# ucb-bar/Accelerated-TinyMPC

Measured on AMD Instinct MI355X. Metric: MPC solves/sec (batched quadrotor nx=12,nu=4,N=30), higher is better.
Workload: dtype f32; 1 GPU; quadrotor_tracking batched 65536 instances per GPU, cold-start tiny_solve, early_exit (tol 1e-3, max_iter 100); nx=12, nu=4, N=30, instances_per_gpu=65536, instances_total=65536, parallelism=batch-shard x1, world_size_seen=1, backend=none (single process), kernel=tile16<12,4,30,exact>, max_iters=85

## Files before the change

accelerated-tinympc_amd/csrc/admm_tile16.hip:

```cpp
#include "rowlane_math.h"
#include <cstdlib>

namespace tinympc
{

typedef float f32x16 __attribute__((ext_vector_type(16)));
#ifndef TINY_T16_ABLATE
#define TINY_T16_ABLATE 0
#endif
#ifndef TINY_T16_CQ
#define TINY_T16_CQ 1
#endif
#ifndef TINY_T16_BADDR
#define TINY_T16_BADDR 1
#endif
#ifndef TINY_T16_PADTAB
#define TINY_T16_PADTAB 1
#endif
#ifndef TINY_T16_XPOSE
#define TINY_T16_XPOSE 1
#endif
#ifndef TINY_T16_SCHED
#define TINY_T16_SCHED 1
#endif
#ifndef TINY_T16_LINES
#define TINY_T16_LINES 1
#endif
#ifndef TINY_T16_STAMP
#define TINY_T16_STAMP 0
#endif

#if TINY_T16_ABLATE == 1
__device__ __forceinline__ f32x4 t16_fake4(float a, float b, f32x4 c) { c[0] += a; c[1] += b; c[2] += a; c[3] += b; return c; }
#define TINY_MFMA4(a, b, c) t16_fake4((a), (b), (c))
#define TINY_MFMA1(a, b, c) __builtin_amdgcn_mfma_f32_16x16x1f32((a), (b), (c), 0, 0, 0)
#else
#define TINY_MFMA4(a, b, c) __builtin_amdgcn_mfma_f32_16x16x4f32((a), (b), (c), 0, 0, 0)
#define TINY_MFMA1(a, b, c) __builtin_amdgcn_mfma_f32_16x16x1f32((a), (b), (c), 0, 0, 0)
#endif

template <int V>
__device__ __forceinline__ void gather12(float (&t)[12], const f32x16 &p0, const f32x16 &p1, const f32x16 &p2)
{
#pragma unroll
    for (int b = 0; b < 4; b++)
    {
        t[b] = p0[4 * b + V];
        t[4 + b] = p1[4 * b + V];
        t[8 + b] = p2[4 * b + V];
    }
}
template <int V>
__device__ __forceinline__ void gather4(float (&t)[4], const f32x16 &p)
{
#pragma unroll
    for (int b = 0; b < 4; b++) t[b] = p[4 * b + V];
}

typedef float f32x2 __attribute__((ext_vector_type(2)));
template <int B>
__device__ __forceinline__ f32x4 blk(const f32x16 &p) { return __builtin_shufflevector(p, p, 4 * B, 4 * B + 1, 4 * B + 2, 4 * B + 3); }
__device__ __forceinline__ void gather12v(f32x4 (&t)[12], const f32x16 &p0, const f32x16 &p1, const f32x16 &p2)
{
    t[0] = blk<0>(p0); t[1] = blk<1>(p0); t[2] = blk<2>(p0); t[3] = blk<3>(p0);
    t[4] = blk<0>(p1); t[5] = blk<1>(p1); t[6] = blk<2>(p1); t[7] = blk<3>(p1);
    t[8] = blk<0>(p2); t[9] = blk<1>(p2); t[10] = blk<2>(p2); t[11] = blk<3>(p2);
}
__device__ __forceinline__ void gather4v(f32x4 (&t)[4], const f32x16 &p)
{
    t[0] = blk<0>(p); t[1] = blk<1>(p); t[2] = blk<2>(p); t[3] = blk<3>(p);
}
template <int LO, int CNT, int NN>
__device__ __forceinline__ f32x4 tree_sum4(const f32x4 (&t)[NN])
{
    if constexpr (CNT == 1) return t[LO];
    else
    {
        constexpr int H = CNT / 2;
        return tree_sum4<LO, H>(t) + tree_sum4<LO + H, CNT - H>(t);
    }
}
template <int PLO, int PCNT, int L, int NN>
__device__ __forceinline__ f32x4 ptree_sum4(const f32x4 (&t)[NN])
{
    if constexpr (PCNT == 1) return t[4 * PLO + L];
    else
    {
        constexpr int H = PCNT / 2;
        return ptree_sum4<PLO, H, L>(t) + ptree_sum4<PLO + H, PCNT - H, L>(t);
    }
}
template <int PLAN, int NN>
__device__ __forceinline__ f32x4 reduce4(const f32x4 (&t)[NN])
{
    if constexpr (NN == 1) return t[0];
    else if constexpr (PLAN == PLAN_SEQ)
    {
        f32x4 acc = t[0];
#pragma unroll
        for (int k = 1; k < NN; k++) acc = acc + t[k];
        return acc;
    }
    else if constexpr (PLAN == PLAN_TREE) return tree_sum4<0, NN>(t);
    else
    {
        static_assert(NN % 4 == 0, "packed VEC plan: whole packets only");
        constexpr int NPK = NN / 4;
        const f32x4 s0 = ptree_sum4<0, NPK, 0>(t), s1 = ptree_sum4<0, NPK, 1>(t), s2 = ptree_sum4<0, NPK, 2>(t), s3 = ptree_sum4<0, NPK, 3>(t);
        return (s0 + s2) + (s1 + s3);
    }
}

template <bool EXACT>
struct TileMath
{
    static constexpr int NX = 12, NU = 4;
    using PL = RowPlans<NX, NU>;
    float A1[3], A2, A3[3], A45, AP[3];
    f32x16 negz;

    __device__ __forceinline__ void load(const float *mats, int g, int c)
    {
        const float *m = mats + 4 * (c & 3) + (c >> 2);
#pragma unroll
        for (int ch = 0; ch < 3; ch++)
        {
            A1[ch] = m[(4 * ch + g) * 16];
            A3[ch] = m[(NX + NU + 4 * ch + g) * 16];
            AP[ch] = m[(2 * NX + 2 * NU + 1 + 4 * ch + g) * 16];
        }
        A2 = m[(NX + g) * 16];
        A45 = m[(2 * NX + NU + g) * 16];
#pragma unroll
        for (int e = 0; e < 16; e++) negz[e] = -0.f;
    }

    struct InFlight
    {
        f32x16 p0, p1, p2, pk;
        f32x4 acc;
    };

    __device__ __forceinline__ void lqr_issue(const float (&s)[3], InFlight &F) const
    {
        if constexpr (EXACT)
        {
            F.p0 = TINY_MFMA1(A1[0], s[0], negz); F.p1 = TINY_MFMA1(A1[1], s[1], negz); F.p2 = TINY_MFMA1(A1[2], s[2], negz);
        }
        else
        {
            f32x4 acc = {-0.f, -0.f, -0.f, -0.f};
            acc = TINY_MFMA4(A1[0], s[0], acc);
            acc = TINY_MFMA4(A1[1], s[1], acc);
            F.acc = TINY_MFMA4(A1[2], s[2], acc);
        }
    }
    __device__ __forceinline__ void lqr_finish(const InFlight &F, float di, float &un, float (&xn)[3]) const
    {
        if constexpr (EXACT)
        {
            static_assert(PL::FWD_XA == PL::FWD_U, "x rows and the u row of a lane are summed in one order (both SEQ for nx = 12, nu = 4)");
            f32x4 t[12];
            gather12v(t, F.p0, F.p1, F.p2);
            const f32x4 acc = reduce4<PL::FWD_XA>(t);
            un = -acc[3] - di;
            const f32x16 pb = TINY_MFMA1(A2, un, negz);
            f32x4 t2[4];
            gather4v(t2, pb);
            const f32x4 xn4 = acc + reduce4<PL::FWD_XB>(t2);
            xn[0] = xn4[0]; xn[1] = xn4[1]; xn[2] = xn4[2];
        }
        else
        {
            un = F.acc[3] - di;
            const f32x4 acc = TINY_MFMA4(A2, un, F.acc);
            xn[0] = acc[0]; xn[1] = acc[1]; xn[2] = acc[2];
        }
    }
    __device__ __forceinline__ void lqr(const float (&s)[3], float di, float &un, float (&xn)[3]) const
    {
        InFlight F;
        lqr_issue(s, F);
        lqr_finish(F, di, un, xn);
    }

    __device__ __forceinline__ void riccati_issue(const float (&p)[3], const f32x4 &lin, InFlight &F) const
    {
        if constexpr (EXACT)
        {
            F.p0 = TINY_MFMA1(A3[0], p[0], negz); F.p1 = TINY_MFMA1(A3[1], p[1], negz); F.p2 = TINY_MFMA1(A3[2], p[2], negz);
            F.pk = TINY_MFMA1(A45, lin[3], negz);
        }
        else
        {
            f32x4 acc = lin;
            acc = TINY_MFMA4(A3[0], p[0], acc);
            acc = TINY_MFMA4(A3[1], p[1], acc);
            F.acc = TINY_MFMA4(A3[2], p[2], acc);
        }
    }
    __device__ __forceinline__ void riccati_finish(const InFlight &F, const f32x4 &lin, float (&pn)[3], float &dd) const
    {
        if constexpr (EXACT)
        {
            f32x4 t4[12];
            gather12v(t4, F.p0, F.p1, F.p2);
            const f32x4 wv = lin + reduce4<PL::BWD_PA>(t4);
            float t[12];
            gather12<3>(t, F.p0, F.p1, F.p2);
            const float wv3 = lin[3] + reduce<PL::BWD_TMP>(t);
            const f32x16 pq = TINY_MFMA1(A45, wv3, negz);
            f32x4 tk4[4];
            gather4v(tk4, F.pk);
            const f32x4 pn4 = wv - reduce4<PL::BWD_PK>(tk4);
            pn[0] = pn4[0]; pn[1] = pn4[1]; pn[2] = pn4[2];
            float tk[4];
            gather4<3>(tk, pq); dd = reduce<PL::BWD_D>(tk);
        }
        else
        {
            const f32x4 nz = {-0.f, -0.f, -0.f, -0.f};
            const f32x4 dq = TINY_MFMA4(A45, F.acc[3], nz);
            const f32x4 acc = TINY_MFMA4(A45, lin[3], F.acc);
            pn[0] = acc[0]; pn[1] = acc[1]; pn[2] = acc[2];
            dd = dq[3];
        }
    }
    __device__ __forceinline__ void riccati(const float (&p)[3], const f32x4 &lin, float (&pn)[3], float &dd) const
    {
        InFlight F;
        riccati_issue(p, lin, F);
        riccati_finish(F, lin, pn, dd);
    }

    __device__ __forceinline__ void terminal(const float (&xr)[3], float (&pt)[3]) const
    {
        if constexpr (EXACT)
        {
            const f32x16 p0 = TINY_MFMA1(AP[0], xr[0], negz), p1 = TINY_MFMA1(AP[1], xr[1], negz), p2 = TINY_MFMA1(AP[2], xr[2], negz);
            float t[12];
            gather12<0>(t, p0, p1, p2); pt[0] = -reduce<PL::TERM>(t);
            gather12<1>(t, p0, p1, p2); pt[1] = -reduce<PL::TERM>(t);
            gather12<2>(t, p0, p1, p2); pt[2] = -reduce<PL::TERM>(t);
        }
        else
        {
            f32x4 acc = {-0.f, -0.f, -0.f, -0.f};
            acc = TINY_MFMA4(AP[0], xr[0], acc);
            acc = TINY_MFMA4(AP[1], xr[1], acc);
            acc = TINY_MFMA4(AP[2], xr[2], acc);
            pt[0] = -acc[0]; pt[1] = -acc[1]; pt[2] = -acc[2];
        }
    }
};

__device__ __forceinline__ float tile_inst_max(float v)
{
    v = fmaxf(v, __shfl_xor(v, 16));
    v = fmaxf(v, __shfl_xor(v, 32));
    return v;
}

__device__ __forceinline__ void acc_put(float &dst, float val) { asm volatile("v_accvgpr_write_b32 %0, %1" : "+a"(dst) : "v"(val)); }
__device__ __forceinline__ float acc_get(const float &src)
{
    float r;
    asm volatile("v_accvgpr_read_b32 %0, %1" : "=v"(r) : "a"(src));
    return r;
}
__device__ __forceinline__ void acc_init(float &dst, float val) { asm volatile("v_accvgpr_write_b32 %0, %1" : "=a"(dst) : "v"(val)); }

typedef __attribute__((address_space(3))) float4 lds_float4;
__device__ __forceinline__ void masked_forward_update(unsigned long long m, float (&a)[4], const f32x4 &tp, float (&bo)[4], const f32x4 &old,
                                                      unsigned sn_addr, const f32x4 &t)
{
    unsigned long long sx;
    asm volatile("s_and_saveexec_b64 %[sx], %[m]\n\t"
                 "v_sub_f32 %[a0], %[p0], %[t0]\n\tv_sub_f32 %[a1], %[p1], %[t1]\n\tv_sub_f32 %[a2], %[p2], %[t2]\n\tv_sub_f32 %[a3], %[p3], %[t3]\n\t"
                 "v_accvgpr_write_b32 %[b0], %[o0]\n\tv_accvgpr_write_b32 %[b1], %[o1]\n\tv_accvgpr_write_b32 %[b2], %[o2]\n\tv_accvgpr_write_b32 %[b3], %[o3]\n\t"
                 "ds_write_b128 %[ad], %[tv]\n\t"
                 "s_mov_b64 exec, %[sx]"
                 : [sx] "=&s"(sx), [a0] "+v"(a[0]), [a1] "+v"(a[1]), [a2] "+v"(a[2]), [a3] "+v"(a[3]), [b0] "+a"(bo[0]), [b1] "+a"(bo[1]),
                   [b2] "+a"(bo[2]), [b3] "+a"(bo[3])
                 : [m] "s"(m), [p0] "v"(tp[0]), [p1] "v"(tp[1]), [p2] "v"(tp[2]), [p3] "v"(tp[3]), [t0] "v"(t[0]), [t1] "v"(t[1]), [t2] "v"(t[2]),
                   [t3] "v"(t[3]), [o0] "v"(old[0]), [o1] "v"(old[1]), [o2] "v"(old[2]), [o3] "v"(old[3]), [ad] "v"(sn_addr), [tv] "v"(t)
                 : "memory", "scc");
}
__device__ __forceinline__ void masked_backward_update(unsigned long long m, float (&pl)[3], float &dr, const float (&pn)[3], float dd)
{
    unsigned long long sx;
    asm volatile("s_and_saveexec_b64 %[sx], %[m]\n\t"
                 "v_accvgpr_write_b32 %[p0], %[n0]\n\tv_accvgpr_write_b32 %[p1], %[n1]\n\tv_accvgpr_write_b32 %[p2], %[n2]\n\tv_mov_b32 %[d], %[dd]\n\t"
                 "s_mov_b64 exec, %[sx]"
                 : [sx] "=&s"(sx), [p0] "+a"(pl[0]), [p1] "+a"(pl[1]), [p2] "+a"(pl[2]), [d] "+v"(dr)
                 : [m] "s"(m), [n0] "v"(pn[0]), [n1] "v"(pn[1]), [n2] "v"(pn[2]), [dd] "v"(dd)
                 : "scc");
}

__device__ __forceinline__ void masked_restore_slack(unsigned long long m, const float (&bo)[4], unsigned sn_addr)
{
    const f32x4 tv = {acc_get(bo[0]), acc_get(bo[1]), acc_get(bo[2]), acc_get(bo[3])};
    unsigned long long sx;
    asm volatile("s_and_saveexec_b64 %[sx], %[m]\n\t"
                 "ds_write_b128 %[ad], %[tv]\n\t"
                 "s_mov_b64 exec, %[sx]"
                 : [sx] "=&s"(sx)
                 : [m] "s"(m), [ad] "v"(sn_addr), [tv] "v"(tv)
                 : "memory", "scc");
}

template <bool EXACT>
__device__ __forceinline__ f32x4 lin_cost4(const f32x4 &cq, const f32x4 &rho4, const f32x4 &t1)
{
    if constexpr (EXACT) return cq - rho4 * t1;
    else return __builtin_elementwise_fma(-rho4, t1, cq);
}

__device__ __forceinline__ f32x4 t16_transpose4(const f32x4 &r)
{
    typedef unsigned u32x2 __attribute__((ext_vector_type(2)));
    const u32x2 a = __builtin_amdgcn_permlane32_swap(__float_as_uint(r[0]), __float_as_uint(r[2]), false, false);
    const u32x2 b = __builtin_amdgcn_permlane32_swap(__float_as_uint(r[1]), __float_as_uint(r[3]), false, false);
    const u32x2 lo = __builtin_amdgcn_permlane16_swap(a[0], b[0], false, false);
    const u32x2 hi = __builtin_amdgcn_permlane16_swap(a[1], b[1], false, false);
    return f32x4{__uint_as_float(lo[0]), __uint_as_float(lo[1]), __uint_as_float(hi[0]), __uint_as_float(hi[1])};
}

constexpr int TILE16_WAVES = 4;
constexpr int TILE16_MAX_TABLE_ROWS = 512;

__device__ __forceinline__ void t16_pair_lines(const f32x4 &e, const f32x4 &o, f32x4 &lo8, f32x4 &hi8)
{
#pragma unroll
    for (int k = 0; k < 4; k++)
    {
        lo8[k] = __int_as_float(__builtin_amdgcn_update_dpp(__float_as_int(e[k]), __float_as_int(o[k]), 0x128, 0xf, 0xc, false));
        hi8[k] = __int_as_float(__builtin_amdgcn_update_dpp(__float_as_int(o[k]), __float_as_int(e[k]), 0x128, 0xf, 0x3, false));
    }
}

#if TINY_T16_STAMP && !defined(TINY_T16_PI_UNIT)
constexpr int T16_STAMP_TILES = 32;
__device__ unsigned long long *t16_stamp_buf;
__device__ int t16_stamp_slots;
__device__ __forceinline__ void t16_stamp(int wslot, int k, int field, unsigned long long v)
{
    unsigned long long *const buf = t16_stamp_buf;
    if (buf && wslot < t16_stamp_slots && k < T16_STAMP_TILES && (threadIdx.x & 63) == 0) buf[((size_t)wslot * T16_STAMP_TILES + k) * 4 + field] = v;
}
#define T16_STAMP(k, field, v) t16_stamp((int)blockIdx.x * TILE16_WAVES + (int)(threadIdx.x >> 6), (k), (field), (v))
#else
#define T16_STAMP(k, field, v) ((void)0)
#endif

__device__ __forceinline__ void t16_dma_row(unsigned on, const float *sbase, unsigned voff, unsigned lds_dst, float after)
{
    asm volatile("s_cmp_eq_u32 %0, 0\n\ts_cbranch_scc1 1f\n\ts_mov_b32 m0, %3\n\ts_nop 0\n\tglobal_load_lds_dwordx4 %1, %2\n1:"
                 : : "s"(on), "v"(voff), "s"(sbase), "s"(lds_dst), "v"(after) : "memory", "scc");
}
__device__ __forceinline__ void t16_dma_row2(unsigned on, const float *sbase, unsigned voff, unsigned lds_dst, float after0, float after1)
{
    asm volatile("s_cmp_eq_u32 %0, 0\n\ts_cbranch_scc1 1f\n\ts_mov_b32 m0, %3\n\ts_nop 0\n\tglobal_load_lds_dwordx4 %1, %2\n\t"
                 "s_add_u32 m0, m0, 0x3f0\n\ts_nop 0\n\tglobal_load_lds_dwordx4 %1, %2 offset:16\n1:"
                 : : "s"(on), "v"(voff), "s"(sbase), "s"(lds_dst), "v"(after0), "v"(after1) : "memory", "scc");
}
__device__ __forceinline__ void t16_dma_img2(unsigned on, const float *sbase, unsigned voff, unsigned lds_dst, float after0, float after1)
{
    asm volatile("s_cmp_eq_u32 %0, 0\n\ts_cbranch_scc1 1f\n\ts_mov_b32 m0, %3\n\ts_nop 0\n\tglobal_load_lds_dwordx4 %1, %2\n\t"
                 "global_load_lds_dwordx4 %1, %2 offset:1024\n1:"
                 : : "s"(on), "v"(voff), "s"(sbase), "s"(lds_dst), "v"(after0), "v"(after1) : "memory", "scc");
}
__device__ __forceinline__ void t16_wait_vm(int k)
{
    if (k == 0) asm volatile("s_waitcnt vmcnt(0)" ::: "memory");
    else if (k == 1) asm volatile("s_waitcnt vmcnt(1)" ::: "memory");
    else if (k == 2) asm volatile("s_waitcnt vmcnt(2)" ::: "memory");
    else if (k == 3) asm volatile("s_waitcnt vmcnt(3)" ::: "memory");
    else if (k == 4) asm volatile("s_waitcnt vmcnt(4)" ::: "memory");
    else if (k == 5) asm volatile("s_waitcnt vmcnt(5)" ::: "memory");
    else if (k == 6) asm volatile("s_waitcnt vmcnt(6)" ::: "memory");
    else if (k == 7) asm volatile("s_waitcnt vmcnt(7)" ::: "memory");
    else asm volatile("s_waitcnt vmcnt(8)" ::: "memory");
}
constexpr int t16_ring_b(bool XR) { return XR ? 3 : 4; }
constexpr int t16_ring_x(bool BR) { return BR ? 4 : 6; }
constexpr int T16_RING_B = 2048, T16_RING_X = 1024;

template <int N, bool EXACT, bool COLD, bool MPC = false, bool BR = false, bool XR = false>
__global__ __launch_bounds__(WAVE * TILE16_WAVES, 1) void admm_tile16_kernel(const RowParams P)
{
    static_assert(!(MPC && (BR || XR)), "the closed loop on chip is instantiated for batch-shared bounds and a shared / windowed reference");
    constexpr int NX = 12, NU = 4;
    const int lane = threadIdx.x & 63, wv = threadIdx.x >> 6, g = lane >> 4, c = lane & 15;
    const int ntiles = (P.batch + 15) >> 4;
    const float rho = P.rho;
    const f32x4 rho4 = {rho, rho, rho, rho};

    extern __shared__ __attribute__((aligned(16))) float4 lds4_base[];
    float4 *const lds4 = lds4_base;
    float4 *const sn0 = lds4 + wv * (N * WAVE) + lane;
    constexpr int DB = t16_ring_b(XR), DX = t16_ring_x(BR);
    const unsigned ringsB = (P.pi_flags & 1u) ? DB : 2, ringsX = (P.pi_flags & 2u) ? DX : 1;
    const unsigned bnd_f4 = BR ? TILE16_WAVES * ringsB * (T16_RING_B / 16) : 2 * N * 4;
    float4 *const blo = lds4 + TILE16_WAVES * N * WAVE, *const bhi = blo + N * 4, *const tab0 = blo + bnd_f4;
    float4 *const tab = tab0;
    const int tab_rows = P.xref_mode == 1 ? P.table_rows : N;
    const float *tab_src = P.xref_mode == 1 ? P.xref_table : P.xref;
    unsigned dmaB = 0, dmaX = 0;
    if constexpr (BR)
    {
        const unsigned ring = (unsigned)(size_t)(lds_float4 *)blo + wv * (ringsB * T16_RING_B);
        dmaB = __builtin_amdgcn_readfirstlane(ring);
    }
    else
    {
        for (int e = threadIdx.x; e < N * 16; e += WAVE * TILE16_WAVES)
        {
            const float2 lh = reinterpret_cast<const float2 *>(P.bounds)[e];
            const int i = e >> 4, r = e & 15;
            reinterpret_cast<float *>(&blo[i * 4 + (r & 3)])[r >> 2] = lh.x;
            reinterpret_cast<float *>(&bhi[i * 4 + (r & 3)])[r >> 2] = lh.y;
        }
    }
    if constexpr (XR)
    {
        const unsigned ring = (unsigned)(size_t)(lds_float4 *)tab0 + wv * (ringsX * T16_RING_X);
        dmaX = __builtin_amdgcn_readfirstlane(ring);
    }
    else
    {
        for (int e = threadIdx.x; e < (tab_rows + N - 1) * 16; e += WAVE * TILE16_WAVES)
        {
            const int er = (e >> 4) < tab_rows ? (e >> 4) : tab_rows - 1;
            float val = tab_src[er * 16 + (e & 15)];
            if (TINY_T16_CQ) val = -(val * ((e & 15) < NX ? P.mats[(2 * NX + 2 * NU) * 16 + (e & 15)] : 1.f));
            reinterpret_cast<float *>(&tab[(e >> 4) * 4 + (e & 3)])[(e & 15) >> 2] = val;
        }
    }
    if constexpr (!BR || !XR) __syncthreads();

    TileMath<EXACT> M;
    M.load(P.mats, g, c);
    f32x4 qv;
#pragma unroll
    for (int v = 0; v < 3; v++) qv[v] = P.mats[(2 * NX + 2 * NU) * 16 + 4 * v + g];
    qv[3] = 1.f;
    constexpr bool CQ = TINY_T16_CQ && !XR;
    auto cost_of = [&](const f32x4 &xr) { return CQ ? xr : -(xr * qv); };

    constexpr bool DQ = COLD && !MPC;
    int qinc = 1;
    if constexpr (DQ)
    {
        const unsigned tail_stride = (P.pi_flags >> 8) & 0xffu;
        if (tail_stride && (((unsigned)blockIdx.x * TILE16_WAVES + (unsigned)wv) % tail_stride) == 0u) qinc = 0x10000;
        qinc = __builtin_amdgcn_readfirstlane(qinc);
    }
#if TINY_T16_STAMP
    int stamp_k = 0;
#else
    constexpr int stamp_k = 0;
#endif
    for (;;)
    {
    int slot = 0;
    if (lane == 0) slot = atomicAdd(P.n_unsolved + 1, qinc);
    slot = __builtin_amdgcn_readfirstlane(slot);
    T16_STAMP(stamp_k, 0, __builtin_amdgcn_s_memrealtime());
    T16_STAMP(stamp_k, 3, ~0ull);
    if (DQ && ntiles <= 32768)
    {
        const int qh = slot & 0xffff, qt = (int)((unsigned)slot >> 16);
        if (qh + qt >= ntiles) break;
        slot = qinc == 1 ? qh : ntiles - 1 - qt;
    }
    else if (slot >= ntiles) break;
    int ozt;
    asm volatile("s_mov_b32 %0, 0" : "=s"(ozt));
    float4 *const sn = sn0 + ozt;
    float4 *const lds4 = lds4_base + ozt;
    int tile = slot;
    if (P.order) tile = P.order[slot];
    const bool tile_ok = tile >= 0 && tile < ntiles;
    T16_STAMP(stamp_k, 3, (unsigned long long)(unsigned)tile);
    constexpr bool GM = COLD && !MPC && !BR && !XR;
    int inst = tile * 16 + c;
    if constexpr (GM)
        if (P.inst_map) inst = P.inst_map[(tile_ok ? tile : 0) * 16 + c];
    auto in_batch = [&](int i) { return GM ? (unsigned)i < (unsigned)P.batch : i < P.batch; };
    const bool valid = tile_ok && in_batch(inst);
    const int inst_a = valid ? inst : P.batch - 1;

    float a[N][4];
    float dr[N], bo[N][4], pl[N][3];
    auto dual4 = [&](int i) { return f32x4{a[i][0], a[i][1], a[i][2], a[i][3]}; };
    const int ebase = (inst_a * N) * 16 + g;
    int wstart = 0;
    if (P.xref_mode == 1) wstart = P.xref_start[inst_a];
    const bool zdual = COLD || (P.duals_zero != 0);

    if constexpr (COLD)
    {
        const float4 z4 = make_float4(0.f, 0.f, 0.f, 0.f);
#pragma unroll
        for (int i = 0; i < N; i++)
        {
            a[i][0] = a[i][1] = a[i][2] = a[i][3] = 0.f;
#pragma unroll
            for (int v = 0; v < 4; v++) acc_init(bo[i][v], 0.f);
            sn[i * WAVE] = z4;
            acc_init(pl[i][0], 0.f); acc_init(pl[i][1], 0.f); acc_init(pl[i][2], 0.f);
            dr[i] = 0.f;
        }
    }
    else
    {
#pragma unroll
        for (int i = 0; i < N; i++)
        {
            float vzl[4], pdv[4];
#pragma unroll
            for (int v = 0; v < 4; v++)
            {
                const int o = ebase + i * 16 + 4 * v;
                vzl[v] = P.vz[o]; pdv[v] = P.pd[o];
                const float gyv = P.gy[o];
                a[i][v] = zdual ? 0.f : gyv;
                acc_init(bo[i][v], vzl[v]);
            }
            sn[i * WAVE] = make_float4(vzl[0], vzl[1], vzl[2], vzl[3]);
            acc_init(pl[i][0], pdv[0]); acc_init(pl[i][1], pdv[1]); acc_init(pl[i][2], pdv[2]);
            dr[i] = pdv[3];
        }
    }
    float x0[3];
#pragma unroll
    for (int v = 0; v < 3; v++) x0[v] = P.xu[ebase + 4 * v];

    const unsigned onB = BR ? (P.pi_flags & 1u) : 0u, onX = XR ? (P.pi_flags & 2u) : 0u;
    struct PiAddr { unsigned rdB, rdX, voffB, voffX; };
    auto pi_addr = [&](unsigned lane16) {
        const unsigned c16 = lane16 & 0xf0u, gg = lane16 >> 8, cc = c16 >> 4;
        const int ins = tile * 16 + (int)cc;
        const unsigned ia = (unsigned)((tile_ok && ins < P.batch) ? ins : P.batch - 1);
        PiAddr A;
        A.rdB = dmaB + 1024u * (gg >> 1) + c16 + 8u * (gg & 1u);
        A.rdX = dmaX + c16 + 4u * gg;
        A.voffB = ia * P.bounds_inst_stride * 8u + 32u * gg;
        A.voffX = ia * P.xref_inst_stride * 4u + 16u * gg;
        return A;
    };
    const float *const xsrc = P.xref;
    auto load_xref = [&](const float4 *tb, int ws, int i, int gsel = -1) {
        if constexpr (XR)
        {
            unsigned ll = lane;
            asm volatile("" : "+v"(ll));
            const unsigned cc = ll & 15u, gg = ll >> 4;
            if (onX)
            {
                const float *rp = xsrc + ((size_t)((tile_ok ? tile : 0) * N + i) * 64 + cc) * 4 + gg;
                return f32x4{rp[0], rp[64], rp[128], 0.f};
            }
            const int ins = tile * 16 + (int)cc;
            const float *rp = xsrc + (size_t)((tile_ok && ins < P.batch) ? ins : P.batch - 1) * P.xref_inst_stride + i * 16 + gg;
            return f32x4{rp[0], rp[4], rp[8], 0.f};
        }
        else
        {
        int row;
        if constexpr (TINY_T16_PADTAB && !(EXACT && COLD && !MPC && !BR && !XR)) row = (ws < tab_rows - 1 ? ws : tab_rows - 1) + i;
        else { row = ws + i; row = row < tab_rows ? row : tab_rows - 1; }
        const float4 t4 = tb[row * 4 + (gsel >= 0 ? gsel : g)];
        return f32x4{t4.x, t4.y, t4.z, t4.w};
        }
    };
    PiAddr A0 = {0u, 0u, 0u, 0u};
    if constexpr (BR || XR)
    {
        A0 = pi_addr(16u * lane);
        if constexpr (BR) { t16_dma_row2(onB ^ 1u, P.bounds, A0.voffB, dmaB, 0.f, 0.f); t16_dma_row2(onB ^ 1u, P.bounds, A0.voffB + (N - 1) * 128u, dmaB + T16_RING_B, 0.f, 0.f); }
        if constexpr (XR) t16_dma_row((onX >> 1) ^ 1u, xsrc, A0.voffX, dmaX, 0.f);
        asm volatile("s_waitcnt vmcnt(0)" ::: "memory");
    }
    auto load_xref_raw = [&](const float4 *tb, int ws, int i) {
        if constexpr (CQ)
        {
            int row = ws + i;
            row = row < tab_rows ? row : tab_rows - 1;
            const float *rp = tab_src + row * 16 + g;
            return f32x4{rp[0], rp[4], rp[8], 0.f};
        }
        else return load_xref(tb, ws, i);
    };
    float pterm[3];
    {
        const f32x4 xrN4 = load_xref_raw(tab, wstart, N - 1);
        const float xrN[3] = {xrN4[0], xrN4[1], xrN4[2]};
        M.terminal(xrN, pterm);
    }

    int st = TINY_STATUS_UNSOLVED_, itn = 1;
    float r_ps = 0.f, r_pi = 0.f, r_ds = 0.f, r_di = 0.f;
    if (valid && !COLD)
    {
        r_ps = P.res[4 * inst + 0]; r_pi = P.res[4 * inst + 1];
        r_ds = P.res[4 * inst + 2]; r_di = P.res[4 * inst + 3];
    }
    float pN[3] = {0.f, 0.f, 0.f};

    auto backward_sweep = [&](unsigned long long amask, const float4 *snI, const float4 *tabI, int wsI) {
        float p[3] = {pN[0], pN[1], pN[2]};
        auto load_lin = [&](int i, float4 &sl, f32x4 &xr) {
            sl = snI[i * WAVE];
            xr = load_xref(tabI, wsI, i);
        };
        auto make_lin = [&](int i, const float4 &sl, const f32x4 &xr) {
            const f32x4 sni = {sl.x, sl.y, sl.z, sl.w};
            return lin_cost4<EXACT>(cost_of(xr), rho4, sni - dual4(i));
        };
        float4 sl0; f32x4 xr0;
        load_lin(N - 2, sl0, xr0);
        f32x4 lin = make_lin(N - 2, sl0, xr0);
#pragma unroll
        for (int i = N - 2; i >= 0; i--)
        {
            float4 sl_n = make_float4(0.f, 0.f, 0.f, 0.f); f32x4 xr_n = {0.f, 0.f, 0.f, 0.f};
            if (EXACT && i > 0) load_lin(i - 1, sl_n, xr_n);
            typename TileMath<EXACT>::InFlight F;
            M.riccati_issue(p, lin, F);
            if (!EXACT && i > 0) load_lin(i - 1, sl_n, xr_n);
#if TINY_T16_SCHED
            if constexpr (EXACT) __builtin_amdgcn_sched_barrier(0);
#endif
            f32x4 lin_n = lin;
            if (i > 0) lin_n = make_lin(i - 1, sl_n, xr_n);
#if TINY_T16_SCHED
            if constexpr (EXACT) __builtin_amdgcn_sched_barrier(0);
#endif
            float pn[3], dd;
            M.riccati_finish(F, lin, pn, dd);
            masked_backward_update(amask, pl[i], dr[i], pn, dd);
            p[0] = pn[0]; p[1] = pn[1]; p[2] = pn[2];
            lin = lin_n;
        }
    };

    for (int ms = 0;; ++ms)
    {
    if (MPC && ms > 0) { st = TINY_STATUS_UNSOLVED_; itn = 1; }
    bool active = valid && (P.max_iter > 0);
    for (int it = 0; it < P.max_iter; ++it)
    {
        if (!__any(active)) break;
        int oz;
        asm volatile("s_mov_b32 %0, 0" : "=s"(oz));
        float4 *const snI = sn + oz;
        const float4 *bloI = blo + oz, *bhiI = bhi + oz;
        const float4 *const tabI = tab + oz;
        const int wsI = wstart + oz;
        const unsigned long long amask = __ballot(active);
        const unsigned sn_addr = (unsigned)(size_t)(lds_float4 *)snI;
        const unsigned gI = (sn_addr - (unsigned)__builtin_amdgcn_readfirstlane(sn_addr)) >> 8;
        const float4 *const bloG = bloI + gI, *const bhiG = bhiI + gI;
        const float *const bsrcI = P.bounds + oz, *const xsrcI = xsrc + oz;
        unsigned rdBI = 0, rdXI = 0;
        if constexpr (BR || XR)
        {
            const PiAddr AI = pi_addr(sn_addr - __builtin_amdgcn_readfirstlane(sn_addr));
            rdBI = COLD ? AI.rdB : A0.rdB + oz; rdXI = COLD ? AI.rdX : A0.rdX + oz;
        }
        const unsigned sB1 = onB ? T16_RING_B : 0u, sX1 = onX ? T16_RING_X : 0u;
        const unsigned sBlast = onB ? ((N - 1) % DB) * T16_RING_B : T16_RING_B;
        const unsigned lane16I = sn_addr - __builtin_amdgcn_readfirstlane(sn_addr);
        const unsigned timg = (unsigned)(tile_ok ? tile : 0) * (unsigned)N;
        unsigned xw = 0, bw = 0;
        if constexpr (XR) xw = timg * 1024u + (COLD ? lane16I : 16u * lane);
        if constexpr (BR) bw = timg * 2048u + (COLD ? lane16I : 16u * lane);
        auto dma_x = [&](int i, float after) { t16_dma_row(onX, xsrcI, xw + (unsigned)i * 1024u, dmaX + (i % DX) * T16_RING_X, after); };
        auto dma_b = [&](int i, float after0, float after1) { t16_dma_img2(onB, bsrcI, bw + (unsigned)i * 2048u, dmaB + (i % DB) * T16_RING_B, after0, after1); };
        typedef __attribute__((address_space(3))) const f32x2 lds_cfloat2;
        typedef __attribute__((address_space(3))) const float lds_cfloat;
        auto ring_bounds = [&](int i, float4 &lo, float4 &hi) {
            lds_cfloat2 *rp = reinterpret_cast<lds_cfloat2 *>(rdBI + (i == N - 1 ? sBlast : (i % DB) * sB1));
            const f32x2 b0 = rp[0], b1 = rp[32], b2 = rp[64], b3 = rp[96];
            lo = make_float4(b0.x, b1.x, b2.x, b3.x); hi = make_float4(b0.y, b1.y, b2.y, b3.y);
        };
        auto ring_xref = [&](int i) {
            lds_cfloat *rp = reinterpret_cast<lds_cfloat *>(rdXI + (i % DX) * sX1);
            return f32x4{rp[0], rp[64], rp[128], 0.f};
        };
        if constexpr (XR)
        {
#pragma unroll
            for (int k = 0; k < DX; k++) dma_x(N - 2 - k, 0.f);
        }
        if constexpr (BR)
        {
#pragma unroll
            for (int k = 0; k < DB - 1; k++) dma_b(k, 0.f, 0.f);
        }
        float s[3] = {x0[0], x0[1], x0[2]};
        float pri_x = 0.f, dua_x = 0.f, pri_u = 0.f, dua_u = 0.f;
        auto elementwise = [&](int i, const f32x4 &sv, const float4 &lo, const float4 &hi, const float4 &ol) {
            const f32x4 old = {ol.x, ol.y, ol.z, ol.w};
            const f32x4 tp = sv + dual4(i);
            f32x4 t;
            t[0] = __builtin_amdgcn_fmed3f(tp[0], lo.x, hi.x);
            t[1] = __builtin_amdgcn_fmed3f(tp[1], lo.y, hi.y);
            t[2] = __builtin_amdgcn_fmed3f(tp[2], lo.z, hi.z);
            t[3] = __builtin_amdgcn_fmed3f(tp[3], lo.w, hi.w);
            const f32x4 dp = sv - t, dd_ = old - t;
            pri_x = fmaxf(fmaxf(fmaxf(pri_x, fabsf(dp[0])), fabsf(dp[1])), fabsf(dp[2]));
            dua_x = fmaxf(fmaxf(fmaxf(dua_x, fabsf(dd_[0])), fabsf(dd_[1])), fabsf(dd_[2]));
            pri_u = fmaxf(pri_u, fabsf(dp[3]));
            dua_u = fmaxf(dua_u, fabsf(dd_[3]));
            if (i == N - 1)
            {
                const f32x4 an = tp - t;
#pragma unroll
                for (int v = 0; v < 3; v++)
                {
                    const float pn_ = lin_cost<EXACT>(pterm[v], rho, t[v] - an[v]);
                    pN[v] = active ? pn_ : pN[v];
                }
            }
            masked_forward_update(amask, a[i], tp, bo[i], old, sn_addr + i * (WAVE * 16), t);
        };
        f32x4 sv_p = {0.f, 0.f, 0.f, 0.f};
        float4 lo_p = make_float4(0.f, 0.f, 0.f, 0.f), hi_p = lo_p, ol_p = lo_p;
#pragma unroll
        for (int i = 0; i < N; i++)
        {
            float4 lo, hi;
            if constexpr (BR)
            {
                if (i + DB - 1 < N) dma_b(i + DB - 1, lo_p.x, hi_p.w);
                t16_wait_vm(2 * ((N - 1 - i) < (DB - 1) ? (N - 1 - i) : (DB - 1)));
                ring_bounds(i, lo, hi);
            }
            else if constexpr (TINY_T16_BADDR && (COLD || !XR)) { lo = bloG[i * 4]; hi = bhiG[i * 4]; }
            else { lo = bloI[i * 4 + g]; hi = bhiI[i * 4 + g]; }
            const float4 ol = snI[i * WAVE];
            typename TileMath<EXACT>::InFlight F;
            if (i < N - 1) M.lqr_issue(s, F);
#if TINY_T16_SCHED
            if constexpr (EXACT) __builtin_amdgcn_sched_barrier(0);
#endif
            if (i > 0) elementwise(i - 1, sv_p, lo_p, hi_p, ol_p);
            float un = 0.f, xn[3] = {0.f, 0.f, 0.f};
            if (i < N - 1) M.lqr_finish(F, dr[i], un, xn);
            sv_p = f32x4{s[0], s[1], s[2], un};
            lo_p = lo; hi_p = hi; ol_p = ol;
            s[0] = xn[0]; s[1] = xn[1]; s[2] = xn[2];
        }
        elementwise(N - 1, sv_p, lo_p, hi_p, ol_p);
        pri_x = tile_inst_max(pri_x); dua_x = tile_inst_max(dua_x);
        pri_u = tile_inst_max(pri_u); dua_u = tile_inst_max(dua_u);
        bool conv = false;
        if (active)
        {
            itn = it + 1;
            if ((it + 1) % P.check_termination == 0)
            {
                r_ps = pri_x; r_ds = dua_x * rho; r_pi = pri_u; r_di = dua_u * rho;
                conv = (r_ps < P.abs_pri_tol) && (r_pi < P.abs_pri_tol) && (r_ds < P.abs_dua_tol) && (r_di < P.abs_dua_tol);
            }
            if (conv) st = TINY_STATUS_SOLVED_;
        }
        active = active && !conv;
        if (!__any(active)) break;
        if (it == P.max_iter - 1) break;
        {
            float p[3] = {pN[0], pN[1], pN[2]};
            const unsigned long long amask = __ballot(active);
            auto load_lin = [&](int i, float4 &sl, f32x4 &xr) {
                sl = snI[i * WAVE];
                if constexpr (XR) xr = ring_xref(i);
                else xr = load_xref(tabI, wsI, i, TINY_T16_BADDR ? (int)gI : -1);
            };
            auto make_lin = [&](int i, const float4 &sl, const f32x4 &xr) {
                const f32x4 sni = {sl.x, sl.y, sl.z, sl.w};
                return lin_cost4<EXACT>(cost_of(xr), rho4, sni - dual4(i));
            };
            float4 sl0; f32x4 xr0;
            if constexpr (XR) t16_wait_vm(0);
            load_lin(N - 2, sl0, xr0);
            f32x4 lin = make_lin(N - 2, sl0, xr0);
#pragma unroll
            for (int i = N - 2; i >= 0; i--)
            {
                float4 sl_n = make_float4(0.f, 0.f, 0.f, 0.f); f32x4 xr_n = {0.f, 0.f, 0.f, 0.f};
                if constexpr (XR)
                {
                    if (i >= DX) dma_x(i - DX, lin[0]);
                    if (i > 0)
                    {
                        const int hi_j = (i - 2) < (N - 2 - DX) ? (i - 2) : (N - 2 - DX), lo_j = (i - DX) > 0 ? (i - DX) : 0;
                        t16_wait_vm(hi_j >= lo_j ? hi_j - lo_j + 1 : 0);
                    }
                }
                if (EXACT && i > 0) load_lin(i - 1, sl_n, xr_n);
                typename TileMath<EXACT>::InFlight F;
                M.riccati_issue(p, lin, F);
                if (!EXACT && i > 0) load_lin(i - 1, sl_n, xr_n);
#if TINY_T16_SCHED
                if constexpr (EXACT) __builtin_amdgcn_sched_barrier(0);
#endif
                f32x4 lin_n = lin;
                if (i > 0) lin_n = make_lin(i - 1, sl_n, xr_n);
#if TINY_T16_SCHED
                if constexpr (EXACT) __builtin_amdgcn_sched_barrier(0);
#endif
                float pn[3], dd;
                M.riccati_finish(F, lin, pn, dd);
                masked_backward_update(amask, pl[i], dr[i], pn, dd);
                p[0] = pn[0]; p[1] = pn[1]; p[2] = pn[2];
                lin = lin_n;
            }
        }
    }
    if (!MPC || ms + 1 >= P.mpc_steps) break;
    if constexpr (MPC)
    {
        int oz;
        asm volatile("s_mov_b32 %0, 0" : "=s"(oz));
        float4 *const snA = sn + oz;
        const unsigned sn_addr = (unsigned)(size_t)(lds_float4 *)snA;
        const bool solved = st == TINY_STATUS_SOLVED_;
        float un, xn_[3];
        M.lqr(x0, dr[0], un, xn_);
        if (P.u0_traj && valid) P.u0_traj[((long long)ms * P.batch + inst) * NU + g] = un;
        {
            const f32x16 p0 = TINY_MFMA1(M.A1[0], x0[0], M.negz), p1 = TINY_MFMA1(M.A1[1], x0[1], M.negz), p2 = TINY_MFMA1(M.A1[2], x0[2], M.negz);
            const f32x16 pb = TINY_MFMA1(M.A2, un, M.negz);
            f32x4 t[12], t2[4];
            gather12v(t, p0, p1, p2);
            gather4v(t2, pb);
            f32x4 z = {0.f, 0.f, 0.f, 0.f};
            asm volatile("" : "+v"(z));
            f32x4 acc = z + t[0];
#pragma unroll
            for (int k = 1; k < 12; k++) acc = acc + t[k];
            const f32x4 x1 = acc + reduce4<PLAN_SEQ>(t2);
            x0[0] = x1[0]; x0[1] = x1[1]; x0[2] = x1[2];
        }
        const unsigned long long umask = __ballot(valid && !solved);
        if (umask != 0ull) backward_sweep(umask, snA, tab + oz, wstart + oz);
        const unsigned long long smask = __ballot(valid && solved);
#pragma unroll
        for (int i = 0; i < N; i++) masked_restore_slack(smask, bo[i], sn_addr + i * (WAVE * 16));
        if (P.xref_mode == 1)
        {
            wstart += P.window_advance;
            const f32x4 xrN4 = load_xref_raw(tab + oz, wstart, N - 1);
            const float xrN[3] = {xrN4[0], xrN4[1], xrN4[2]};
            M.terminal(xrN, pterm);
        }
#pragma unroll
        for (int i = 0; i < N; i++) a[i][0] = a[i][1] = a[i][2] = a[i][3] = 0.f;
    }
    }
    T16_STAMP(stamp_k, 1, __builtin_amdgcn_s_memrealtime());

    auto inst_of = [&](int col) {
        if constexpr (GM)
        {
            int tl = tile_ok ? tile : 0;
            asm volatile("" : "+s"(tl));
            if (P.inst_map) return P.inst_map[tl * 16 + col];
            return tl * 16 + col;
        }
        else return tile * 16 + col;
    };
    int inst_e = inst, ebase_e = ebase;
    bool valid_e = valid;
    if constexpr (GM)
    {
        unsigned ll = lane;
        asm volatile("" : "+v"(ll));
        inst_e = inst_of((int)(ll & 15u));
        valid_e = tile_ok && in_batch(inst_e);
        ebase_e = ((valid_e ? inst_e : P.batch - 1) * N) * 16 + (int)(ll >> 4);
    }

    if (P.max_iter <= 0)
    {
        if (valid_e && g == 0)
        {
            P.status[inst_e] = TINY_STATUS_UNSOLVED_;
            P.iter[inst_e] = 1;
            atomicAdd(P.n_unsolved, 1);
        }
        T16_STAMP(stamp_k, 2, __builtin_amdgcn_s_memrealtime());
#if TINY_T16_STAMP
        ++stamp_k;
#endif
        continue;
    }

    {
        const bool solved = st == TINY_STATUS_SOLVED_;
        const int c2 = lane >> 2, q2 = lane & 3;
        const int inst2 = inst_of(c2);
        const bool valid2 = tile_ok && in_batch(inst2);
        const int obase2 = ((valid2 ? inst2 : 0) * N) * 16 + 4 * q2;
        typedef float float_ma __attribute__((may_alias));
        typedef f32x4 f32x4_ma __attribute__((may_alias));
        float_ma *const stage_w = reinterpret_cast<float_ma *>(lds4 + wv * (N * WAVE));
        const int rd_off = (c2 * 4 + q2);
        const int obase4 = ebase_e + 3 * g;
        constexpr bool XPOSE = TINY_T16_XPOSE && !(EXACT && !COLD && !MPC);
        auto put = [&](float *dst, int i, const f32x4 &val) {
            if constexpr (XPOSE)
            {
                const f32x4 o = t16_transpose4(val);
                if (valid_e) *reinterpret_cast<f32x4 *>(dst + obase4 + i * 16) = o;
                return;
            }
            float_ma *slot = stage_w + i * (WAVE * 4);
            reinterpret_cast<f32x4_ma *>(slot)[lane] = val;
            asm volatile("" ::: "memory");
            f32x4 o;
            o[0] = slot[rd_off]; o[1] = slot[rd_off + 64]; o[2] = slot[rd_off + 128]; o[3] = slot[rd_off + 192];
            asm volatile("" ::: "memory");
            if (valid2) *reinterpret_cast<f32x4 *>(dst + obase2 + i * 16) = o;
        };
        float s[3] = {x0[0], x0[1], x0[2]};
        if constexpr (XPOSE && TINY_T16_LINES && COLD && !MPC && !BR && !XR)
        {
            auto slack_of = [&](int i) { return reinterpret_cast<const f32x4_ma *>(stage_w + i * (WAVE * 4))[lane]; };
            auto lin_of = [&](int i, const f32x4 &sni) {
                const f32x4 xr = load_xref(tab, wstart, i);
                f32x4 lin = lin_cost4<EXACT>(cost_of(xr), rho4, sni - dual4(i));
                if (i == N - 1) lin[3] = 0.f;
                return lin;
            };
            auto pd_of = [&](int i) { return i == N - 1 ? f32x4{pN[0], pN[1], pN[2], 0.f} : f32x4{acc_get(pl[i][0]), acc_get(pl[i][1]), acc_get(pl[i][2]), dr[i]}; };
            auto vz_of = [&](int i, const f32x4 &sni) {
                f32x4 vzv;
    #pragma unroll
                for (int v = 0; v < 4; v++)
                {
                    const float bov = acc_get(bo[i][v]);
                    vzv[v] = solved ? bov : sni[v];
                }
                return vzv;
            };
            const int instL = inst_of(c & 7), instH = inst_of((c & 7) + 8);
            const bool validL = tile_ok && in_batch(instL), validH = tile_ok && in_batch(instH);
            const int obaseL = (validL ? instL : 0) * (N * 16) + ((c >> 3) << 4) + 4 * g;
            const int offH = ((validH ? instH : 0) - (validL ? instL : 0)) * (N * 16);
            auto put2 = [&](float *dst, int i, const f32x4 &ve, const f32x4 &vo) {
                f32x4 lo8, hi8;
                t16_pair_lines(t16_transpose4(ve), t16_transpose4(vo), lo8, hi8);
                if (validL) *reinterpret_cast<f32x4 *>(dst + obaseL + i * 16) = lo8;
                if (validH) *reinterpret_cast<f32x4 *>(dst + obaseL + offH + i * 16) = hi8;
            };
#pragma unroll
            for (int i = 0; i + 1 < N; i += 2)
            {
                const f32x4 sne = slack_of(i), sno = slack_of(i + 1);
                put2(P.gy, i, dual4(i), dual4(i + 1));
                put2(P.vzn, i, sne, sno);
                put2(P.vz, i, vz_of(i, sne), vz_of(i + 1, sno));
                put2(P.pd, i, pd_of(i), pd_of(i + 1));
                put2(P.qr, i, lin_of(i, sne), lin_of(i + 1, sno));
                float ue = 0.f, xe[3];
                M.lqr(s, dr[i], ue, xe);
                const f32x4 sve = {s[0], s[1], s[2], ue};
                float uo = 0.f, xo[3] = {0.f, 0.f, 0.f};
                if (i + 1 < N - 1) M.lqr(xe, dr[i + 1], uo, xo);
                put2(P.xu, i, sve, f32x4{xe[0], xe[1], xe[2], uo});
                s[0] = xo[0]; s[1] = xo[1]; s[2] = xo[2];
            }
            if constexpr (N % 2 == 1)
            {
                const f32x4 sni = slack_of(N - 1);
                put(P.xu, N - 1, f32x4{s[0], s[1], s[2], 0.f});
                put(P.qr, N - 1, lin_of(N - 1, sni));
                put(P.pd, N - 1, pd_of(N - 1));
                put(P.vz, N - 1, vz_of(N - 1, sni));
                put(P.vzn, N - 1, sni);
                put(P.gy, N - 1, dual4(N - 1));
            }
        }
        else
        {
#pragma unroll
        for (int i = 0; i < N; i++)
        {
            float un = 0.f, xn[3] = {0.f, 0.f, 0.f};
            if (i < N - 1) M.lqr(s, dr[i], un, xn);
            const f32x4 sv = {s[0], s[1], s[2], un};
            const f32x4 sni = reinterpret_cast<const f32x4_ma *>(stage_w + i * (WAVE * 4))[lane];
            const f32x4 xr = load_xref(tab, wstart, i);
            f32x4 lin = lin_cost4<EXACT>(cost_of(xr), rho4, sni - dual4(i));
            if (i == N - 1) lin[3] = 0.f;
            f32x4 pdv = {acc_get(pl[i][0]), acc_get(pl[i][1]), acc_get(pl[i][2]), dr[i]};
            if (i == N - 1) pdv = f32x4{pN[0], pN[1], pN[2], 0.f};
            f32x4 vzv;
#pragma unroll
            for (int v = 0; v < 4; v++)
            {
                const float bov = acc_get(bo[i][v]);
                vzv[v] = solved ? bov : sni[v];
            }
            put(P.xu, i, sv);
            put(P.qr, i, lin);
            put(P.pd, i, pdv);
            put(P.vz, i, vzv);
            put(P.vzn, i, sni);
            put(P.gy, i, dual4(i));
            if constexpr (!XPOSE) reinterpret_cast<f32x4_ma *>(stage_w + i * (WAVE * 4))[lane] = sni;
            s[0] = xn[0]; s[1] = xn[1]; s[2] = xn[2];
        }
        }
        const unsigned long long umask = __ballot(valid_e && !solved);
        if (umask != 0ull)
        {
            const bool unsolved2 = valid2 && ((umask >> c2) & 1ull);
            float p[3] = {pN[0], pN[1], pN[2]};
#pragma unroll
            for (int i = N - 2; i >= 0; i--)
            {
                const f32x4 sni = reinterpret_cast<const f32x4_ma *>(stage_w + i * (WAVE * 4))[lane];
                const f32x4 xr = load_xref(tab, wstart, i);
                const f32x4 lin = lin_cost4<EXACT>(cost_of(xr), rho4, sni - dual4(i));
                float pn[3], dd;
                M.riccati(p, lin, pn, dd);
                if constexpr (XPOSE)
                {
                    const f32x4 o = t16_transpose4(f32x4{pn[0], pn[1], pn[2], dd});
                    if (valid_e && !solved) *reinterpret_cast<f32x4 *>(P.pd + obase4 + i * 16) = o;
                }
                else
                {
                float_ma *slot = stage_w + i * (WAVE * 4);
                reinterpret_cast<f32x4_ma *>(slot)[lane] = f32x4{pn[0], pn[1], pn[2], dd};
                asm volatile("" ::: "memory");
                f32x4 o;
                o[0] = slot[rd_off]; o[1] = slot[rd_off + 64]; o[2] = slot[rd_off + 128]; o[3] = slot[rd_off + 192];
                asm volatile("" ::: "memory");
                if (unsolved2) *reinterpret_cast<f32x4 *>(P.pd + obase2 + i * 16) = o;
                }
                p[0] = pn[0]; p[1] = pn[1]; p[2] = pn[2];
            }
        }
        if (valid_e && g == 0)
        {
            P.res[4 * inst_e + 0] = r_ps; P.res[4 * inst_e + 1] = r_pi;
            P.res[4 * inst_e + 2] = r_ds; P.res[4 * inst_e + 3] = r_di;
            P.status[inst_e] = st;
            P.iter[inst_e] = itn;
            if (!solved) atomicAdd(P.n_unsolved, 1);
        }
        if (MPC && valid)
        {
#pragma unroll
            for (int v = 0; v < 3; v++) P.x0buf[inst * NX + 4 * v + g] = x0[v];
            if (g == 0 && P.xref_mode == 1) P.xref_start[inst] = wstart;
        }
    }
    T16_STAMP(stamp_k, 2, __builtin_amdgcn_s_memrealtime());
#if TINY_T16_STAMP
    ++stamp_k;
#endif
    }
}

#ifdef TINY_T16_ONLY30
#define TINY_FOR_EACH_TILE16(X) X(30)
#else
#define TINY_FOR_EACH_TILE16(X) X(30) X(25) X(20) X(10)
#endif

static inline unsigned t16_tail_stride(const RowParams &P, int ntiles, int nblocks, int asked, bool grouped)
{
    static const int env = [] { const char *e = getenv("TINYMPC_T16_TAIL"); return e ? atoi(e) : -1; }();
    const int forced = asked >= 0 ? asked : env;
    if (ntiles > 32768) return 0u;
    if (forced >= 0) return (P.cold_start && P.mpc_steps <= 1) ? (unsigned)(forced > 255 ? 255 : forced) : 0u;
    if (!P.order || P.mpc_steps > 1 || !P.cold_start) return 0u;
    const int slots = nblocks * TILE16_WAVES;
    if (ntiles < 3 * slots) return 0u;
    if (grouped) return ntiles < 8 * slots ? 12u : 8u;
    return (ntiles >= 4 * slots && ntiles < 8 * slots) ? 4u : 8u;
}

#ifdef TINY_T16_PI_UNIT
size_t tile16_pi_lds_bytes(int N, bool bounds_ring, bool xref_ring, unsigned pi_flags, int table_rows)
{
    const size_t bnd = bounds_ring ? (size_t)TILE16_WAVES * ((pi_flags & 1u) ? t16_ring_b(xref_ring) : 2) * T16_RING_B : (size_t)2 * N * 4 * sizeof(float4);
    const size_t ref = xref_ring ? (size_t)TILE16_WAVES * ((pi_flags & 2u) ? t16_ring_x(bounds_ring) : 1) * T16_RING_X : (size_t)(table_rows + N - 1) * 4 * sizeof(float4);
    return (size_t)TILE16_WAVES * N * WAVE * sizeof(float4) + bnd + ref;
// ... 124 lines not shown
```

Before: 48.04 million solves/s.

## Interleave per-row MFMA issue with loads in forward and backward sweeps

Adds a new scheduling mode (default SCHED=2) for the exact cold-start path. It splits the LQR forward and Riccati backward MFMA issues into individual instructions and places sched barriers between them so global loads and elementwise work fill the MFMA latency. The backward loop defers part of the step-1 update and the linear-cost construction into the step-0 iteration using a carry struct, and adds a held finish variant with asm register pins. This raises code complexity and risks scheduling conflicts or register pressure from the fixed ordering.

```diff
diff --git a/accelerated-tinympc_amd/csrc/admm_tile16.hip b/accelerated-tinympc_amd/csrc/admm_tile16.hip
--- a/accelerated-tinympc_amd/csrc/admm_tile16.hip
+++ b/accelerated-tinympc_amd/csrc/admm_tile16.hip
@@ -21,8 +21,9 @@
 #define TINY_T16_XPOSE 1
 #endif
 #ifndef TINY_T16_SCHED
-#define TINY_T16_SCHED 1
-#endif
+#define TINY_T16_SCHED 2
+#endif
+#define T16_FENCE() __builtin_amdgcn_sched_barrier(0)
 #ifndef TINY_T16_LINES
 #define TINY_T16_LINES 1
 #endif
@@ -176,6 +177,37 @@
             const f32x4 acc = TINY_MFMA4(A2, un, F.acc);
             xn[0] = acc[0]; xn[1] = acc[1]; xn[2] = acc[2];
         }
+    }
+    template <int K>
+    __device__ __forceinline__ void lqr_issue1(const float (&s)[3], InFlight &F) const
+    {
+        if constexpr (K == 0) F.p0 = TINY_MFMA1(A1[0], s[0], negz);
+        else if constexpr (K == 1) F.p1 = TINY_MFMA1(A1[1], s[1], negz);
+        else F.p2 = TINY_MFMA1(A1[2], s[2], negz);
+    }
+    __device__ __forceinline__ f32x4 lqr_finish_u(InFlight &F, float di, float &un) const
+    {
+        f32x4 t[12];
+        gather12v(t, F.p0, F.p1, F.p2);
+        const f32x4 acc = reduce4<PL::FWD_XA>(t);
+        un = -acc[3] - di;
+        F.pk = TINY_MFMA1(A2, un, negz);
+        return acc;
+    }
+    __device__ __forceinline__ void lqr_finish_x(const InFlight &F, const f32x4 &acc, float (&xn)[3]) const
+    {
+        f32x4 t2[4];
+        gather4v(t2, F.pk);
+        const f32x4 xn4 = acc + reduce4<PL::FWD_XB>(t2);
+        xn[0] = xn4[0]; xn[1] = xn4[1]; xn[2] = xn4[2];
+    }
+    template <int K>
+    __device__ __forceinline__ void riccati_issue1(const float (&p)[3], float r, InFlight &F) const
+    {
+        if constexpr (K == 0) F.p0 = TINY_MFMA1(A3[0], p[0], negz);
+        else if constexpr (K == 1) F.p1 = TINY_MFMA1(A3[1], p[1], negz);
+        else if constexpr (K == 2) F.p2 = TINY_MFMA1(A3[2], p[2], negz);
+        else F.pk = TINY_MFMA1(A45, r, negz);
     }
     __device__ __forceinline__ void lqr(const float (&s)[3], float di, float &un, float (&xn)[3]) const
     {
@@ -226,6 +258,28 @@
             dd = dq[3];
         }
     }
+    __device__ __forceinline__ void riccati_finish_hold(const InFlight &F, const f32x4 &lin, float (&pn)[3], float &dd) const
+    {
+        f32x4 t4[12];
+        gather12v(t4, F.p0, F.p1, F.p2);
+        const f32x4 wv = lin + reduce4<PL::BWD_PA>(t4);
+        float t[12];
+        gather12<3>(t, F.p0, F.p1, F.p2);
+        const float wv3 = lin[3] + reduce<PL::BWD_TMP>(t);
+        const f32x16 pq = TINY_MFMA1(A45, wv3, negz);
+        f32x16 pkh = F.pk;
+        T16_FENCE();
+        asm volatile("" : "+v"(pkh));
+        f32x4 tk4[4];
+        gather4v(tk4, pkh);
+        const f32x4 pn4 = wv - reduce4<PL::BWD_PK>(tk4);
+        pn[0] = pn4[0]; pn[1] = pn4[1]; pn[2] = pn4[2];
+        asm volatile("" : "+v"(pn[0]), "+v"(pn[1]), "+v"(pn[2]));
+        T16_FENCE();
+        asm volatile("" : : "v"(pq));
+        float tk[4];
+        gather4<3>(tk, pq); dd = reduce<PL::BWD_D>(tk);
+    }
     __device__ __forceinline__ void riccati(const float (&p)[3], const f32x4 &lin, float (&pn)[3], float &dd) const
     {
         InFlight F;
@@ -325,6 +379,17 @@
     const u32x2 hi = __builtin_amdgcn_permlane16_swap(a[1], b[1], false, false);
     return f32x4{__uint_as_float(lo[0]), __uint_as_float(lo[1]), __uint_as_float(hi[0]), __uint_as_float(hi[1])};
 }
+
+template <bool ON>
+struct T16Carry
+{
+    float dd = 0.f;
+    float lm[3] = {0.f, 0.f, 0.f}, lc[3] = {0.f, 0.f, 0.f};
+};
+template <>
+struct T16Carry<false>
+{
+};
 
 constexpr int TILE16_WAVES = 4;
 constexpr int TILE16_MAX_TABLE_ROWS = 512;
@@ -484,6 +549,7 @@
     const bool tile_ok = tile >= 0 && tile < ntiles;
     T16_STAMP(stamp_k, 3, (unsigned long long)(unsigned)tile);
     constexpr bool GM = COLD && !MPC && !BR && !XR;
+    constexpr bool IL = (TINY_T16_SCHED >= 2) && EXACT && GM;
     int inst = tile * 16 + c;
     if constexpr (GM)
         if (P.inst_map) inst = P.inst_map[(tile_ok ? tile : 0) * 16 + c];
@@ -608,6 +674,7 @@
         r_ds = P.res[4 * inst + 2]; r_di = P.res[4 * inst + 3];
     }
     float pN[3] = {0.f, 0.f, 0.f};
+    T16Carry<IL> cr;
 
     auto backward_sweep = [&](unsigned long long amask, const float4 *snI, const float4 *tabI, int wsI) {
         float p[3] = {pN[0], pN[1], pN[2]};
@@ -733,6 +800,48 @@
         for (int i = 0; i < N; i++)
         {
             float4 lo, hi;
+            if constexpr (IL)
+            {
+                if (i < N - 1)
+                {
+                    typename TileMath<EXACT>::InFlight F;
+                    float4 ol;
+                    float un = 0.f, xn[3] = {0.f, 0.f, 0.f};
+                    if (i == 0)
+                    {
+                        const float2 *lp = reinterpret_cast<const float2 *>(bloG);
+                        T16_FENCE();
+                        M.template lqr_issue1<0>(s, F); T16_FENCE();
+                        const float2 la = lp[0]; T16_FENCE();
+                        M.template lqr_issue1<1>(s, F); T16_FENCE();
+                        const float2 lb = lp[1]; T16_FENCE();
+                        M.template lqr_issue1<2>(s, F); T16_FENCE();
+                        hi = bhiG[0]; T16_FENCE();
+                        lo = make_float4(la.x, la.y, lb.x, lb.y);
+                        const f32x4 acc = M.lqr_finish_u(F, dr[0], un);
+                        T16_FENCE();
+                        ol = snI[0];
+                        T16_FENCE();
+                        M.lqr_finish_x(F, acc, xn);
+                    }
+                    else
+                    {
+                        T16_FENCE();
+                        M.template lqr_issue1<0>(s, F); T16_FENCE();
+                        lo = bloG[i * 4]; T16_FENCE();
+                        M.template lqr_issue1<1>(s, F); T16_FENCE();
+                        hi = bhiG[i * 4]; T16_FENCE();
+                        M.template lqr_issue1<2>(s, F); T16_FENCE();
+                        ol = snI[i * WAVE]; T16_FENCE();
+                        elementwise(i - 1, sv_p, lo_p, hi_p, ol_p);
+                        M.lqr_finish(F, dr[i], un, xn);
+                    }
+                    sv_p = f32x4{s[0], s[1], s[2], un};
+                    lo_p = lo; hi_p = hi; ol_p = ol;
+                    s[0] = xn[0]; s[1] = xn[1]; s[2] = xn[2];
+                    continue;
+                }
+            }
             if constexpr (BR)
             {
                 if (i + DB - 1 < N) dma_b(i + DB - 1, lo_p.x, hi_p.w);
@@ -791,6 +900,52 @@
             for (int i = N - 2; i >= 0; i--)
             {
                 float4 sl_n = make_float4(0.f, 0.f, 0.f, 0.f); f32x4 xr_n = {0.f, 0.f, 0.f, 0.f};
+                if constexpr (IL)
+                {
+                    typename TileMath<EXACT>::InFlight F;
+                    f32x4 lin_n = lin;
+                    const float2 *xp = reinterpret_cast<const float2 *>(tabI);
+                    if (i > 0)
+                    {
+                        int row = wsI + i - 1;
+                        row = row < tab_rows ? row : tab_rows - 1;
+                        xp = reinterpret_cast<const float2 *>(tabI + row * 4 + (int)gI);
+                    }
+                    float2 xa = make_float2(0.f, 0.f), xb = xa;
+                    T16_FENCE();
+                    M.template riccati_issue1<0>(p, lin[3], F); T16_FENCE();
+                    if (i > 0) sl_n = snI[(i - 1) * WAVE];
+                    else masked_backward_update(amask, pl[1], dr[1], p, cr.dd);
+                    T16_FENCE();
+                    M.template riccati_issue1<1>(p, lin[3], F); T16_FENCE();
+                    if (i > 0) xa = xp[0];
+                    else lin[0] = cr.lc[0] - cr.lm[0];
+                    T16_FENCE();
+                    M.template riccati_issue1<2>(p, lin[3], F); T16_FENCE();
+                    if (i > 0) xb = xp[1];
+                    else lin[1] = cr.lc[1] - cr.lm[1];
+                    T16_FENCE();
+                    M.template riccati_issue1<3>(p, lin[3], F); T16_FENCE();
+                    xr_n = f32x4{xa.x, xa.y, xb.x, xb.y};
+                    if (i > 1) lin_n = make_lin(i - 1, sl_n, xr_n);
+                    else if (i == 1)
+                    {
+                        const f32x4 cq = cost_of(xr_n);
+                        const float m0 = rho * (sl_n.x - a[0][0]), m1 = rho * (sl_n.y - a[0][1]), m2 = rho * (sl_n.z - a[0][2]), m3 = rho * (sl_n.w - a[0][3]);
+                        lin_n[3] = cq[3] - m3;
+                        cr.lm[0] = m0; cr.lm[1] = m1; cr.lm[2] = m2; cr.lc[0] = cq[0]; cr.lc[1] = cq[1]; cr.lc[2] = cq[2];
+                    }
+                    else lin[2] = cr.lc[2] - cr.lm[2];
+                    T16_FENCE();
+                    float pn[3], dd;
+                    if (i == 0) M.riccati_finish_hold(F, lin, pn, dd);
+                    else M.riccati_finish(F, lin, pn, dd);
+                    if (i != 1) masked_backward_update(amask, pl[i], dr[i], pn, dd);
+                    p[0] = pn[0]; p[1] = pn[1]; p[2] = pn[2];
+                    cr.dd = dd;
+                    lin = lin_n;
+                    continue;
+                }
                 if constexpr (XR)
                 {
                     if (i >= DX) dma_x(i - DX, lin[0]);
```

Result: slower. 47.54 million solves/s (-1.0%).
